# dremovd/PPO

Measured on AMD Instinct MI355X. Metric: env-steps/sec (Pong-shaped synthetic, 256 envs/GPU), higher is better.
Workload: dtype f32

## Files before the change

ppo_amd/csrc/stack_fused.hip:

```cpp
#include <cstdlib>
#include <type_traits>

#include "common.h"
#include "conv_stage.h"
#include "mfma.h"

#ifndef PPO_TAIL_SPLIT
#define PPO_TAIL_SPLIT 2
#endif

namespace ppo {
namespace {

constexpr int kScrPitchS = 20;

struct StackTailArgs {
    const float *in;
    const float *w[4];
    const float *bias[4];
    const float *mask[4];
    float *save[4];
    int n_images;
};

// ... 291 lines not shown

            __syncthreads();
#pragma unroll 1
            for (int hs = 0; hs <= S::NBANDS; ++hs) {
                if ((hs & 1) == grp) {
                    if (hs < S::NBANDS) {
                        const int y0 = hs * TR;
                        const int chan_off = ch * (H * W) + y0 * W;
#pragma unroll
                        for (int m = 0; m < MT; ++m) {
                            const bool live = p4[m] < S::NPIX;
                            const int off = live ? (chan_off + p4[m]) * 4 : kOutside;
                            if constexpr (BACKWARD) gate4[m] = buffer_f32x4(mask_b, off);
                            res4[m] = buffer_f32x4(res_b, off);
                        }
                        constexpr int CS_HI = ((C / 4 - 1) * 4 * PLANE + 2 * PITCH + 2) * 4 > 65535 ? C / 8 : C / 4;
                        static_assert(((C / 4 - 1 - (CS_HI < C / 4 ? CS_HI : 0)) * 4 * PLANE + 2 * PITCH + 2) * 4 <= 65535 &&
                                      ((CS_HI - 1) * 4 * PLANE + 2 * PITCH + 2) * 4 <= 65535, "operand offsets fit the instruction");
                        using lds_cvf = const volatile __attribute__((address_space(3))) float;
                        lds_cvf *vsmem = (lds_cvf *)smem;
                        int base[MT], base_hi[MT];
#pragma unroll
                        for (int m = 0; m < MT; ++m) {
                            base[m] = lofs[m] + (y0 - 1 + in_row) * PITCH;
                            base_hi[m] = base[m] + CS_HI * 4 * PLANE;
                            if constexpr (CS_HI < C / 4) asm volatile("" : "+v"(base_hi[m]));
                            acc[m] = f32x4{0.f, 0.f, 0.f, 0.f};
                        }
                        constexpr int SB = 2;
                        constexpr int NB = (KS + SB - 1) / SB;
                        float raw[2][SB][MT];
                        auto load_block = [&](int j, float (&r)[SB][MT]) {
#pragma unroll
                            for (int u = 0; u < SB; ++u) {
                                const int s = j * SB + u;
                                if (s < KS) {
                                    const int tap = s / (C / 4), cs = s % (C / 4);
                                    const int tap_off = (tap / 3) * PITCH + (tap % 3);
#pragma unroll
                                    for (int m = 0; m < MT; ++m)
                                        r[u][m] = cs < CS_HI ? vsmem[base[m] + cs * 4 * PLANE + tap_off]
                                                             : vsmem[base_hi[m] + (cs - CS_HI) * 4 * PLANE + tap_off];
                                }
                            }
                        };
                        load_block(0, raw[0]);
#pragma unroll
                        for (int j = 0; j < NB; ++j) {
                            __builtin_amdgcn_sched_barrier(0);
                            if (j + 1 < NB) load_block(j + 1, raw[(j + 1) & 1]);
                            __builtin_amdgcn_sched_barrier(0);
#pragma unroll
                            for (int u = 0; u < SB; ++u) {
                                const int s = j * SB + u;
                                if (s < KS) {
#pragma unroll
                                    for (int m = 0; m < MT; ++m) acc[m] = mfma16(wa[s], raw[j & 1][u][m], acc[m]);
                                }
                            }
                            __builtin_amdgcn_sched_barrier(0);
                        }
                    } else if (layer < 3) {
                        for (int i = tid % (S::GW * 64); i < C * W; i += S::GW * 64)
                            smem[(i / W) * PLANE + G + (H + in_row - 1) * PITCH + i % W] = 0.f;
                    }
                } else if (hs >= 1) {
                    const int y0 = (hs - 1) * TR;
                    const int chan_off = ch * (H * W) + y0 * W;
#pragma unroll
                    for (int m = 0; m < MT; ++m)
#pragma unroll
                        for (int r = 0; r < 4; ++r) scr[(m * 16 + g * 4 + r) * kScrPitchS + l15] = acc[m][r];
                    __builtin_amdgcn_wave_barrier();
                    float *out_row = smem + ch * PLANE + G + (y0 + in_row - 1) * PITCH;
#pragma unroll
                    for (int m = 0; m < MT; ++m) {
                        if (p4[m] >= S::NPIX) continue;
                        const float4 o = *reinterpret_cast<const float4 *>(scr + (m * 16 + ch) * kScrPitchS + quad * 4);
                        const float ov[4] = {o.x, o.y, o.z, o.w};
                        const float gv[4] = {gate4[m].x, gate4[m].y, gate4[m].z, gate4[m].w};
                        const float rv[4] = {res4[m].x, res4[m].y, res4[m].z, res4[m].w};
                        float v[4];
#pragma unroll
                        for (int e = 0; e < 4; ++e) {
                            float val = ov[e] + bias_c;
                            if constexpr (BACKWARD) val = gv[e] > 0.f ? val : 0.f;
                            v[e] = val + rv[e];
                        }
                        if (layer < 3) {
                            float t[4];
#pragma unroll
                            for (int e = 0; e < 4; ++e) t[e] = BACKWARD ? v[e] : relu1(v[e]);
                            *reinterpret_cast<float2 *>(out_row + po[m][0]) = make_float2(t[0], t[1]);
                            *reinterpret_cast<float2 *>(out_row + po[m][1]) = make_float2(t[2], t[3]);
                        }
                        if (save) *reinterpret_cast<float4 *>(save + chan_off + p4[m]) = make_float4(v[0], v[1], v[2], v[3]);
                    }
                    __builtin_amdgcn_wave_barrier();
                }
                __syncthreads();
            }
        }
    }
}

template <int C, int H, int W, int TR, bool BACKWARD>
int launch_stack_shift(const StackTailArgs &args, hipStream_t st)
{
    using S = ShiftCfg<C, H, W, TR>;
    constexpr auto kern = stack_shift_kernel<C, H, W, TR, BACKWARD>;
    if (int rc = prepare_kernel<kern>("stack_shift", S::LDS_BYTES)) return rc;
    int grid = 256;
    if (grid > args.n_images) grid = args.n_images;
    hipLaunchKernelGGL(kern, dim3(grid), dim3(S::NW * 64), S::LDS_BYTES, st, args);
    return check_launch("stack_shift_kernel");
}

template <int I, int N, class F>
__device__ __forceinline__ void static_for(F &&f)
{
    if constexpr (I < N) {
        f(std::integral_constant<int, I>{});
        static_for<I + 1, N>(f);
    }
}

struct LaneMap {
    template <int MT>
    struct T {
        int pix[MT], lofs[MT];
        float hi_l[MT], hi_r[MT];
    };
};

template <int H, int W, int PLANE, int G, int MT, int PITCH = W>
__device__ __forceinline__ void lane_map_init(LaneMap::T<MT> &lm, int pixel_wave, int l15, int g)
{
#pragma unroll
    for (int m = 0; m < MT; ++m) {
        const int p = (pixel_wave * MT + m) * 16 + l15;
        lm.pix[m] = p;
        const int pc = p < H * W ? p : 0;
        if constexpr (PITCH == W) {
            lm.lofs[m] = G + pc - 1 + g * PLANE;
            lm.hi_l[m] = (pc % W == 0) ? 0.f : INFINITY;
            lm.hi_r[m] = (pc % W == W - 1) ? 0.f : INFINITY;
        } else {
            lm.lofs[m] = G + (pc / W) * PITCH + pc % W - 1 + g * PLANE;
            lm.hi_l[m] = lm.hi_r[m] = 0.f;
        }
    }
}

template <int C, int H, int W, int MT, int NTOT, int NT, bool RELU_IN, bool GATED = false, int PITCH = W>
__device__ __forceinline__ void resident_conv(float *smem, int src_off, int dst_off, bool residual, const float *wpk,
                                              const float *bias, float *save, const LaneMap::T<MT> &lm, int n0, int lane,
                                              const float *mask = nullptr)
{
    constexpr int ROWS = H + 2, G = 4, PLANE_RAW = ROWS * PITCH + 2 * G;
    constexpr int PLANE = PLANE_RAW + ((16 - PLANE_RAW % 32) + 32) % 32;
    constexpr int KS = 9 * (C / 4);
    constexpr bool PADDED = PITCH != W;
    static_assert(!PADDED || (PITCH == W + 1 && !RELU_IN), "padded maps hold what the MFMA takes: identity input only");
    const int g = lane >> 4;
    float wa[NT][KS];
    const float4 *pw = reinterpret_cast<const float4 *>(wpk);
#pragma unroll
    for (int s4 = 0; s4 < KS / 4; ++s4)
#pragma unroll
        for (int n = 0; n < NT; ++n) {
            const float4 v = pw[(s4 * NTOT + n0 + n) * 64 + lane];
            wa[n][4 * s4 + 0] = v.x;
            wa[n][4 * s4 + 1] = v.y;
            wa[n][4 * s4 + 2] = v.z;
            wa[n][4 * s4 + 3] = v.w;
        }
    float bias_r[NT][4];
#pragma unroll
    for (int n = 0; n < NT; ++n)
#pragma unroll
        for (int r = 0; r < 4; ++r) bias_r[n][r] = (GATED || !bias) ? 0.f : bias[(n0 + n) * 16 + g * 4 + r];
    constexpr int SB = (MT * NT >= 4) ? 2 : 4;
    constexpr int NB = (KS + SB - 1) / SB;
    constexpr int GATE_AT = (GATED && MT * NT * 4 > 16) ? NB / 2 : -1;
    float gate[GATED ? MT : 1][NT][4];
    auto load_gate = [&]() {
        const __amdgpu_buffer_rsrc_t mask_b = buffer_of(mask);
#pragma unroll
        for (int m = 0; m < MT; ++m)
#pragma unroll
            for (int n = 0; n < NT; ++n)
#pragma unroll
                for (int r = 0; r < 4; ++r)
                    gate[m][n][r] = buffer_f32(mask_b, lm.pix[m] < H * W ? (((n0 + n) * 16 + g * 4 + r) * (H * W) + lm.pix[m]) * 4
                                                                         : kOutside);
    };
    if constexpr (GATED && GATE_AT < 0) load_gate();

    __syncthreads();
    int base[MT];
#pragma unroll
    for (int m = 0; m < MT; ++m) {
        base[m] = lm.lofs[m] + src_off;
        if constexpr (PADDED) asm volatile("" : "+v"(base[m]));
    }
    f32x4 acc[NT][MT];
#pragma unroll
    for (int n = 0; n < NT; ++n)
#pragma unroll
        for (int m = 0; m < MT; ++m) acc[n][m] = f32x4{0.f, 0.f, 0.f, 0.f};

    float raw[2][SB][MT];
    auto load_block = [&](int j, float (&r)[SB][MT]) {
#pragma unroll
        for (int u = 0; u < SB; ++u) {
            const int s = j * SB + u;
            if (s < KS) {
                const int tap = s / (C / 4), cs = s % (C / 4);
                const int tap_off = (tap / 3) * PITCH + (tap % 3);
#pragma unroll
                for (int m = 0; m < MT; ++m) {
                    if constexpr (PADDED) {
                        using lds_cvf = const volatile __attribute__((address_space(3))) float;
                        r[u][m] = ((lds_cvf *)smem)[base[m] + cs * 4 * PLANE + tap_off];
                    } else {
                        r[u][m] = smem[base[m] + cs * 4 * PLANE + tap_off];
                    }
                }
            }
        }
    };
    static_assert(!PADDED || ((C / 4 - 1) * 4 * PLANE + 2 * PITCH + 2) * 4 <= 65535, "operand offsets fit the instruction");
    load_block(0, raw[0]);
    static_for<0, NB>([&](auto jc) {
        constexpr int j = decltype(jc)::value;
        float bv[SB][MT];
#pragma unroll
        for (int u = 0; u < SB; ++u) {
            const int s = j * SB + u;
            if (s < KS) {
                const int kx = (s / (C / 4)) % 3;
#pragma unroll
                for (int m = 0; m < MT; ++m) {
                    float x = raw[j & 1][u][m];
                    if constexpr (PADDED) {
                    } else if (kx != 1) {
                        const float hi = kx == 0 ? lm.hi_l[m] : lm.hi_r[m];
                        x = __builtin_amdgcn_fmed3f(x, RELU_IN ? 0.f : -hi, hi);
                    } else if (RELU_IN) {
                        x = relu1(x);
                    }
                    bv[u][m] = x;
                }
            }
        }
        __builtin_amdgcn_sched_barrier(0);
        if constexpr (j + 1 < NB) load_block(j + 1, raw[(j + 1) & 1]);
        if constexpr (PADDED) __builtin_amdgcn_sched_barrier(0);
        if constexpr (j == GATE_AT) load_gate();
#pragma unroll
        for (int u = 0; u < SB; ++u) {
            const int s = j * SB + u;
            if (s < KS) {
#pragma unroll
                for (int m = 0; m < MT; ++m)
#pragma unroll
                    for (int n = 0; n < NT; ++n) acc[n][m] = mfma16(wa[n][s], bv[u][m], acc[n][m]);
            }
        }
        __builtin_amdgcn_sched_barrier(0);
    });
#pragma unroll
    for (int m = 0; m < MT; ++m) {
        if (lm.pix[m] < H * W) {
#pragma unroll
            for (int n = 0; n < NT; ++n)
#pragma unroll
                for (int r = 0; r < 4; ++r) {
                    const int co = (n0 + n) * 16 + g * 4 + r;
                    const int lo = PADDED ? dst_off + co * PLANE + (lm.lofs[m] - g * PLANE) + PITCH + 1
                                          : dst_off + co * PLANE + G + W + lm.pix[m];
                    float val = acc[n][m][r] + bias_r[n][r];
                    if constexpr (GATED) val = gate[m][n][r] > 0.f ? val : 0.f;
                    if (residual) val = val + smem[lo];
                    smem[lo] = val;
                    if (save) save[(size_t)co * (H * W) + lm.pix[m]] = val;
                }
        }
    }
}

struct StackFullArgs {
    const float *in;
    const float *w[5];
    const float *bias[5];
    float *pooled;
    uint8_t *argmax;
    float *save[4];
    const float *pre_w[4];
    const float *pre_bias[4];
    float *pre_save[4];
    int has_pre;
    int n_images;
};

template <int C, int HI, int WI, int MTI, int HO, int WO, int MTO, int NW, int NSPLIT>
__global__ __launch_bounds__(NW * NSPLIT * 64) void stack_full_kernel(StackFullArgs a)
{
    using SI = StackCfg<C, HI, WI, MTI, NW, NSPLIT>;
    using SO = StackCfg<C, HO, WO, MTO, NW, NSPLIT>;
    static_assert(HO == (HI + 1) / 2 && WO == (WI + 1) / 2, "3x3 / stride 2 / pad 1 pooling");
    static_assert(2 * SO::LDS_MAP <= SI::LDS_MAP, "the small maps reuse the input map's LDS");
    constexpr int NT = SI::NTL, WAVES = SI::WAVES, THREADS = WAVES * 64;
    constexpr int A_OFF = 0, B_OFF = SI::LDS_MAP, X_OFF = 0, Y_OFF = SO::LDS_MAP;
    extern __shared__ __align__(16) float smem[];
    const int tid = threadIdx.x, lane = tid & 63, l15 = lane & 15, g = lane >> 4;
    const int wave = tid >> 6, pixel_wave = wave % NW, n0 = (wave / NW) * NT;

    LaneMap::T<MTI> lmi;
    LaneMap::T<MTO> lmo;
    lane_map_init<HI, WI, SI::PLANE, SI::G, MTI>(lmi, pixel_wave, l15, g);
    lane_map_init<HO, WO, SO::PLANE, SO::G, MTO>(lmo, pixel_wave, l15, g);

    if (a.has_pre) zero_lds<SI::LDS_MAP, THREADS>(smem + B_OFF, tid);

    for (int img = blockIdx.x; img < a.n_images; img += gridDim.x) {
        __syncthreads();
        zero_lds<SI::LDS_MAP, THREADS>(smem + A_OFF, tid);
        __syncthreads();
        stage_band_chunk_dma<C, HI, WI, SI::ROWS, SI::PLANE, SI::G, WAVES>(a.in, img, 0, smem + A_OFF, tid);
        if (a.has_pre) {
            const size_t big_img = (size_t)img * C * HI * WI;
#pragma unroll 1
            for (int layer = 0; layer < 4; ++layer) {
                const int odd = layer & 1;
                float *save = a.pre_save[layer] ? a.pre_save[layer] + big_img : nullptr;
                resident_conv<C, HI, WI, MTI, SI::NT, NT, true>(smem, odd ? B_OFF : A_OFF, odd ? A_OFF : B_OFF, odd != 0,
                                                                a.pre_w[layer], a.pre_bias[layer], save, lmi, n0, lane);
            }
        }
        resident_conv<C, HI, WI, MTI, SI::NT, NT, false>(smem, A_OFF, B_OFF, false, a.w[0], a.bias[0], nullptr, lmi, n0, lane);
        __syncthreads();
        zero_lds<2 * SO::LDS_MAP, THREADS>(smem + X_OFF, tid);
        __syncthreads();
        {
            constexpr int RPW = 64 / WO;
            const int sub = lane / WO, xo = lane % WO;
            const size_t out_img = (size_t)img * C * HO * WO;
            for (int u0 = wave * RPW; u0 < C * HO; u0 += WAVES * RPW) {
                const int u = u0 + sub;
                const int co = u / HO, yo = u % HO;
                if (sub < RPW && co < C) {
                    const float *src = smem + B_OFF + co * SI::PLANE + SI::G + WI + (2 * yo - 1) * WI + 2 * xo - 1;
                    float best;
                    int best_tap;
                    pool_window_lds<HI % 2 == 0, WI % 2 == 0>(src, WI, yo > 0, 2 * yo + 1 < HI, xo > 0, 2 * xo + 1 < WI, best, best_tap);
                    smem[X_OFF + co * SO::PLANE + SO::G + WO + yo * WO + xo] = best;
                    const size_t oi = out_img + ((size_t)co * HO + yo) * WO + xo;
                    if (a.pooled) a.pooled[oi] = best;
                    if (a.argmax) a.argmax[oi] = (uint8_t)best_tap;
                }
            }
        }
        const size_t out_img = (size_t)img * C * HO * WO;
#pragma unroll 1
        for (int layer = 0; layer < 4; ++layer) {
            const int odd = layer & 1;
            float *save = a.save[layer] ? a.save[layer] + out_img : nullptr;
            resident_conv<C, HO, WO, MTO, SO::NT, NT, true>(smem, odd ? Y_OFF : X_OFF, odd ? X_OFF : Y_OFF, odd != 0,
                                                            a.w[1 + layer], a.bias[1 + layer], save, lmo, n0, lane);
        }
    }
}

struct StackFullBwdArgs {
    const float *g;
    const float *w[5];
    const float *mask[4];
    const uint8_t *argmax;
    float *save[4];
    float *dc;
    float *g_prev;
    const float *post_w[4];
    const float *post_mask[4];
    float *post_save[4];
    int has_post;
    int n_images;
};

template <int C, int HI, int WI, int MTI, int HO, int WO, int MTO, int NW, int NSPLIT>
__global__ __launch_bounds__(NW * NSPLIT * 64) void stack_full_bwd_kernel(StackFullBwdArgs a)
{
    using SI = StackCfg<C, HI, WI, MTI, NW, NSPLIT, WI + 1>;
    using SO = StackCfg<C, HO, WO, MTO, NW, NSPLIT, WO + 1>;
    static_assert(2 * SO::LDS_MAP <= SI::LDS_MAP, "the small maps live inside the first big map's LDS");
    static_assert(C * HO * WO <= SO::LDS_MAP * 4, "the argmax bytes of an image fit the second small map");
    constexpr int NT = SI::NTL, WAVES = SI::WAVES, THREADS = WAVES * 64;
    constexpr int A_OFF = 0, B_OFF = SI::LDS_MAP, X_OFF = 0, Y_OFF = SO::LDS_MAP;
    extern __shared__ __align__(16) float smem[];
    const int tid = threadIdx.x, lane = tid & 63, l15 = lane & 15, g = lane >> 4;
    const int wave = tid >> 6, pixel_wave = wave % NW, n0 = (wave / NW) * NT;

    LaneMap::T<MTI> lmi;
    LaneMap::T<MTO> lmo;
    lane_map_init<HI, WI, SI::PLANE, SI::G, MTI, SI::PITCH>(lmi, pixel_wave, l15, g);
    lane_map_init<HO, WO, SO::PLANE, SO::G, MTO, SO::PITCH>(lmo, pixel_wave, l15, g);

    zero_lds<SI::LDS_MAP, THREADS>(smem + B_OFF, tid);

    for (int img = blockIdx.x; img < a.n_images; img += gridDim.x) {
        __syncthreads();
        zero_lds<2 * SO::LDS_MAP, THREADS>(smem + X_OFF, tid);
        __syncthreads();
        const size_t small_img = (size_t)img * C * HO * WO, big_img = (size_t)img * C * HI * WI;
        for (int row = tid; row < C * HO; row += THREADS) {
            const float *gr = a.g + small_img + row * WO;
            float *lr = smem + X_OFF + (row / HO) * SO::PLANE + SO::G + (1 + row % HO) * SO::PITCH;
            float gv[WO];
#pragma unroll
            for (int x = 0; x < WO; ++x) gv[x] = gr[x];
#pragma unroll
            for (int x = 0; x < WO; ++x) lr[x] = gv[x];
        }
        constexpr int AM_WORDS = C * HO * WO / 4, AM_PER = (AM_WORDS + THREADS - 1) / THREADS;
        static_assert(C * HO * WO % 4 == 0, "an image's argmax bytes are whole words (the entry points check the base)");
        uint32_t am_r[AM_PER];
#pragma unroll
        for (int k = 0; k < AM_PER; ++k) {
            const int i = tid + k * THREADS;
            am_r[k] = reinterpret_cast<const uint32_t *>(a.argmax + small_img)[i < AM_WORDS ? i : 0];
        }
#pragma unroll 1
        for (int layer = 0; layer < 4; ++layer) {
            const int odd = layer & 1;
            resident_conv<C, HO, WO, MTO, SO::NT, NT, false, true, SO::PITCH>(smem, odd ? Y_OFF : X_OFF, odd ? X_OFF : Y_OFF, odd != 0,
                                                                   a.w[layer], nullptr, a.save[layer] + small_img, lmo, n0,
                                                                   lane, a.mask[layer] + small_img);
        }
        __syncthreads();
        const uint8_t *am = reinterpret_cast<const uint8_t *>(smem + Y_OFF);
#pragma unroll
        for (int k = 0; k < AM_PER; ++k) {
            const int i = tid + k * THREADS;
            if (i < AM_WORDS) reinterpret_cast<uint32_t *>(smem + Y_OFF)[i] = am_r[k];
        }
        __syncthreads();
        {
            for (int e = tid; e < C * HI * WI; e += THREADS) {
                const int co = e / (HI * WI), r = e % (HI * WI);
                const int iy = r / WI, ix = r % WI;
                const int k = ix >> 1, oy0 = iy >> 1;
                const int ky0 = (iy & 1) ? 2 : 1;
                const bool has_oy1 = (iy & 1) && (oy0 + 1 < HO);
                const bool odd_x = ix & 1;
                const bool has_ox1 = odd_x && (k + 1 < WO);
                const int kx0 = odd_x ? 2 : 1;
                const float *gx = smem + X_OFF + co * SO::PLANE + SO::G + SO::PITCH;
                const uint8_t *ac = am + co * (HO * WO);
                float sum = 0.f;
                {
                    const int i00 = oy0 * WO + k, x00 = oy0 * SO::PITCH + k;
                    if (ac[i00] == ky0 * 3 + kx0) sum += gx[x00];
                    if (has_ox1 && ac[i00 + 1] == ky0 * 3 + 0) sum += gx[x00 + 1];
                }
                if (has_oy1) {
                    const int i10 = (oy0 + 1) * WO + k, x10 = (oy0 + 1) * SO::PITCH + k;
                    if (ac[i10] == kx0) sum += gx[x10];
                    if (has_ox1 && ac[i10 + 1] == 0) sum += gx[x10 + 1];
                }
                smem[B_OFF + co * SI::PLANE + SI::G + (1 + iy) * SI::PITCH + ix] = sum;
                a.dc[big_img + e] = sum;
            }
        }
        if (a.has_post) {
            __syncthreads();
            zero_lds<SI::LDS_MAP, THREADS>(smem + A_OFF, tid);
        }
        resident_conv<C, HI, WI, MTI, SI::NT, NT, false, false, SI::PITCH>(smem, B_OFF, A_OFF, false, a.w[4], nullptr,
                                                                a.g_prev + big_img, lmi, n0, lane);
        if (a.has_post) {
#pragma unroll 1
            for (int layer = 0; layer < 4; ++layer) {
                const int odd = layer & 1;
                resident_conv<C, HI, WI, MTI, SI::NT, NT, false, true, SI::PITCH>(smem, odd ? B_OFF : A_OFF, odd ? A_OFF : B_OFF, odd != 0,
                                                                       a.post_w[layer], nullptr, a.post_save[layer] + big_img,
                                                                       lmi, n0, lane, a.post_mask[layer] + big_img);
            }
        }
    }
}

template <int C, int HI, int WI, int MTI, int HO, int WO, int MTO, int NW, int NSPLIT>
int launch_stack_full(const StackFullBwdArgs &args, hipStream_t st)
{
    using SI = StackCfg<C, HI, WI, MTI, NW, NSPLIT, WI + 1>;
    constexpr size_t kLds = 2 * (size_t)SI::LDS_MAP * 4;
    static_assert(kLds <= 160 * 1024, "two padded maps fit the CU's LDS");
    constexpr auto kern = stack_full_bwd_kernel<C, HI, WI, MTI, HO, WO, MTO, NW, NSPLIT>;
    if (int rc = prepare_kernel<kern>("stack_full_bwd", kLds)) return rc;
    const int grid = args.n_images < 256 ? args.n_images : 256;
    hipLaunchKernelGGL(kern, dim3(grid), dim3(SI::WAVES * 64), kLds, st, args);
    return check_launch("stack_full_bwd_kernel");
}

template <int C, int HI, int WI, int MTI, int HO, int WO, int MTO, int NW, int NSPLIT>
int launch_stack_full(const StackFullArgs &args, hipStream_t st)
{
    using SI = StackCfg<C, HI, WI, MTI, NW, NSPLIT>;
    constexpr size_t kLds = 2 * (size_t)SI::LDS_MAP * 4;
    constexpr auto kern = stack_full_kernel<C, HI, WI, MTI, HO, WO, MTO, NW, NSPLIT>;
    if (int rc = prepare_kernel<kern>("stack_full", kLds)) return rc;
    const int grid = args.n_images < 256 ? args.n_images : 256;
    hipLaunchKernelGGL(kern, dim3(grid), dim3(SI::WAVES * 64), kLds, st, args);
    return check_launch("stack_full_kernel");
}


struct ChainSplitArgs {
    const float *in;
    const float *pre_w[4];
    const float *pre_bias[4];
    const float *w[5];
    const float *bias[5];
    float *out;
    float *xbuf;
    uint32_t *flags;
    uint32_t *ctl;
    int n_images;
    int skip;
};

constexpr int kSplitWaves = 8;
constexpr uint32_t kSpinLimit = 1u << 21;

template <int C, int HI, int WI, int HO, int WO>
__global__ __launch_bounds__(kSplitWaves * 64) void stack_chain_split_kernel(ChainSplitArgs a)
{
    static_assert(C == 32, "two channel tiles: one per workgroup of a pair");
    using SI = StackCfg<C, HI, WI, 7, 4, 2>;
    using SO = StackCfg<C, HO, WO, 2, 4, 2>;
    constexpr int MTI = 4, MTO = 2, WAVES = kSplitWaves, THREADS = WAVES * 64;
    static_assert(SI::MTILES <= MTI * WAVES && SO::MTILES == MTO * 4 && WAVES == 8, "every pixel tile has a wave");
    static_assert(2 * SO::LDS_MAP <= SI::LDS_MAP, "the small maps reuse the input map's LDS");
    constexpr int A_OFF = 0, B_OFF = SI::LDS_MAP, X_OFF = 0, Y_OFF = SO::LDS_MAP;
    extern __shared__ __align__(16) float smem[];
    const int tid = threadIdx.x, lane = tid & 63, l15 = lane & 15, g = lane >> 4;
    const int wave = tid >> 6;
    const int b = blockIdx.x;
    const int h = (b >> 3) & 1;
    const int pair0 = (b & 7) | ((b >> 4) << 3);
    const int n_pairs = (gridDim.x >> 4) << 3;

    LaneMap::T<MTI> lmi;
    LaneMap::T<MTO> lmo;
    lane_map_init<HI, WI, SI::PLANE, SI::G, MTI>(lmi, wave, l15, g);
    lane_map_init<HO, WO, SO::PLANE, SO::G, MTO>(lmo, wave & 3, l15, g);

    const uint32_t base = __hip_atomic_load(a.ctl, __ATOMIC_RELAXED, __HIP_MEMORY_SCOPE_AGENT) * 8u;
    const uint32_t fault = __hip_atomic_load(a.ctl + 3, __ATOMIC_RELAXED, __HIP_MEMORY_SCOPE_AGENT);
    const uint32_t spin_limit = fault ? 1u << 10 : kSpinLimit;
    bool gave_up = false;
    zero_lds<SI::LDS_MAP, THREADS>(smem + B_OFF, tid);

    for (int img = pair0; img < a.n_images; img += n_pairs) {
        uint32_t *flag_own = a.flags + 2 * img + h, *flag_other = a.flags + 2 * img + (1 - h);
        float *slots = a.xbuf + (size_t)img * 2 * C * HI * WI;
        uint32_t step = 0;
        auto exchange = [&](int dst_off, float *slot, bool fetch) {
            ++step;
            asm volatile("s_waitcnt vmcnt(0)" ::: "memory");
            __syncthreads();
            if (tid == 0) {
                if (!(fault && h == 1))
                    __hip_atomic_store(flag_own, base + step, __ATOMIC_RELAXED, __HIP_MEMORY_SCOPE_AGENT);
                uint32_t it = 0;
                while (!(a.skip & 1) && !gave_up &&
                       __hip_atomic_load(flag_other, __ATOMIC_RELAXED, __HIP_MEMORY_SCOPE_AGENT) < base + step) {
                    if (++it > spin_limit ||
                        ((it & 1023u) == 0 && __hip_atomic_load(a.ctl + 2, __ATOMIC_RELAXED, __HIP_MEMORY_SCOPE_AGENT))) {
                        __hip_atomic_store(a.ctl + 2, 1u, __ATOMIC_RELAXED, __HIP_MEMORY_SCOPE_AGENT);
                        gave_up = true;
                        break;
                    }
                    __builtin_amdgcn_s_sleep(2);
                }
            }
            __syncthreads();
            if (fetch)
                stage_band_chunk_dma<16, HI, WI, SI::ROWS, SI::PLANE, SI::G, WAVES, 16>(slot + (size_t)(1 - h) * 16 * HI * WI, 0, 0,
                                                                                       smem + dst_off + (1 - h) * 16 * SI::PLANE, tid);
        };

        __syncthreads();
        zero_lds<SI::LDS_MAP, THREADS>(smem + A_OFF, tid);
        __syncthreads();
        stage_band_chunk_dma<C, HI, WI, SI::ROWS, SI::PLANE, SI::G, WAVES>(a.in, img, 0, smem + A_OFF, tid);
#pragma unroll 1
        for (int layer = 0; layer < 4; ++layer) {
            const int odd = layer & 1;
            float *slot = slots + (size_t)(layer & 1) * C * HI * WI;
            resident_conv<C, HI, WI, MTI, 2, 1, true>(smem, odd ? B_OFF : A_OFF, odd ? A_OFF : B_OFF, odd != 0, a.pre_w[layer],
                                                      a.pre_bias[layer], slot, lmi, h, lane);
            exchange(odd ? A_OFF : B_OFF, slot, true);
        }
        resident_conv<C, HI, WI, MTI, 2, 1, false>(smem, A_OFF, B_OFF, false, a.w[0], a.bias[0], slots, lmi, h, lane);
        exchange(B_OFF, slots, h == 0);
        if (h != 0 || (a.skip & 2)) continue;
        __syncthreads();
        zero_lds<2 * SO::LDS_MAP, THREADS>(smem + X_OFF, tid);
        __syncthreads();
        {
            constexpr int RPW = 64 / WO;
            const int sub = lane / WO, xo = lane % WO;
            for (int u0 = wave * RPW; u0 < C * HO; u0 += WAVES * RPW) {
                const int u = u0 + sub;
                const int co = u / HO, yo = u % HO;
                if (sub < RPW && co < C) {
                    const float *src = smem + B_OFF + co * SI::PLANE + SI::G + WI + (2 * yo - 1) * WI + 2 * xo - 1;
                    float best;
                    int best_tap;
                    pool_window_lds<HI % 2 == 0, WI % 2 == 0>(src, WI, yo > 0, 2 * yo + 1 < HI, xo > 0, 2 * xo + 1 < WI, best, best_tap);
                    smem[X_OFF + co * SO::PLANE + SO::G + WO + yo * WO + xo] = best;
                }
            }
        }
        float *out_img = a.out + (size_t)img * C * HO * WO;
#pragma unroll 1
        for (int layer = 0; layer < 4; ++layer) {
            const int odd = layer & 1;
            resident_conv<C, HO, WO, MTO, 2, 1, true>(smem, odd ? Y_OFF : X_OFF, odd ? X_OFF : Y_OFF, odd != 0, a.w[1 + layer],
                                                      a.bias[1 + layer], layer == 3 ? out_img : nullptr, lmo, wave >> 2, lane);
        }
    }
    __syncthreads();
    if (tid == 0) {
        const uint32_t done = __hip_atomic_fetch_add(a.ctl + 1, 1u, __ATOMIC_RELAXED, __HIP_MEMORY_SCOPE_AGENT);
        if (done == gridDim.x - 1) {
            __hip_atomic_store(a.ctl + 1, 0u, __ATOMIC_RELAXED, __HIP_MEMORY_SCOPE_AGENT);
            __hip_atomic_fetch_add(a.ctl, 1u, __ATOMIC_RELAXED, __HIP_MEMORY_SCOPE_AGENT);
        }
    }
}

template <int C, int HI, int WI, int HO, int WO>
int launch_chain_split(const ChainSplitArgs &args, hipStream_t st)
{
    using SI = StackCfg<C, HI, WI, 7, 4, 2>;
    constexpr size_t kLds = 2 * (size_t)SI::LDS_MAP * 4;
    constexpr auto kern = stack_chain_split_kernel<C, HI, WI, HO, WO>;
    if (int rc = prepare_kernel<kern>("stack_chain_split", kLds)) return rc;
    int groups = (args.n_images + 7) / 8;
    if (groups > 16) groups = 16;
    hipLaunchKernelGGL(kern, dim3(16 * groups), dim3(kSplitWaves * 64), kLds, st, args);
    return check_launch("stack_chain_split_kernel");
}

#define PPO_STACK_CASE(LAUNCH, C, H, W, ...) \
    if (channels == C && h == H && w == W) return args ? LAUNCH<C, H, W, __VA_ARGS__>(*args, st) : PPO_OK;

int no_kernel(const char *who, int channels, int h, int w)
{
    return fail(PPO_E_INVALID, "%s: no kernel for %d channels at %dx%d", who, channels, h, w);
}

template <bool BACKWARD>
int dispatch_stack_tail(const char *who, int channels, int h, int w, const StackTailArgs *args, hipStream_t st)
{
    PPO_STACK_CASE(launch_stack_shift, 16, 42, 42, 6, BACKWARD)
    PPO_STACK_CASE(launch_stack_shift, 16, 32, 32, 8, BACKWARD)
    PPO_STACK_CASE(launch_stack_tail, 32, 11, 11, 2, 4, PPO_TAIL_SPLIT, BACKWARD)
    PPO_STACK_CASE(launch_stack_tail, 32, 21, 21, 7, 4, PPO_TAIL_SPLIT, BACKWARD)
    PPO_STACK_CASE(launch_stack_tail, 32, 16, 16, 4, 4, PPO_TAIL_SPLIT, BACKWARD)
    PPO_STACK_CASE(launch_stack_tail, 32, 8, 8, 1, 4, PPO_TAIL_SPLIT, BACKWARD)
    return args ? no_kernel(who, channels, h, w) : PPO_E_INVALID;
}

template <class Args>
int dispatch_stack_full(const char *who, int channels, int h, int w, const Args *args, hipStream_t st)
{
    PPO_STACK_CASE(launch_stack_full, 32, 21, 21, 7, 11, 11, 2, 4, 2)
    PPO_STACK_CASE(launch_stack_full, 32, 16, 16, 4, 8, 8, 1, 4, 2)
    return args ? no_kernel(who, channels, h, w) : PPO_E_INVALID;
}

int dispatch_chain_split(const char *who, int channels, int h, int w, const ChainSplitArgs *args, hipStream_t st)
{
    PPO_STACK_CASE(launch_chain_split, 32, 21, 21, 11, 11)
    return args ? no_kernel(who, channels, h, w) : PPO_E_INVALID;
}
#undef PPO_STACK_CASE

template <int N, int M>
int fill_layers(const char *who, const char *other, const float *const *weights, const float *const *others,
                const float *(&w)[N], const float *(&o)[M])
{
    for (int l = 0; l < N; ++l) {
        if (!weights[l] || (l < M && !others[l])) return fail(PPO_E_INVALID, "%s: null weights / %s of layer %d", who, other, l);
        if (!aligned(weights[l], 16)) return fail(PPO_E_ALIGN, "%s: packed weights must be 16-byte aligned", who);
        w[l] = weights[l];
        if (l < M) o[l] = others[l];
    }
    return PPO_OK;
}

struct ChainedStack {
    const float *const *weights, *const *others;
    float *save[4];
};

int stack_full_forward(const char *who, const float *in, const ChainedStack *pre, const float *const *packed_weights,
                       const float *const *biases, float *pooled, uint8_t *argmax, float *a0, float *q0, float *a1, float *q1,
                       int n_images, int channels, int h, int w, void *stream)
{
    if (n_images < 0) return fail(PPO_E_INVALID, "%s: negative batch", who);
    if (n_images == 0) return PPO_OK;
    if (!in || !packed_weights || !biases || !q1 || (pre && (!pre->weights || !pre->others)))
        return fail(PPO_E_INVALID, "%s: null pointer", who);
    StackFullArgs args{};
    args.in = in, args.pooled = pooled, args.argmax = argmax, args.n_images = n_images;
    args.save[0] = a0, args.save[1] = q0, args.save[2] = a1, args.save[3] = q1;
    if (int rc = fill_layers(who, "bias", packed_weights, biases, args.w, args.bias)) return rc;
    if (pre) {
        if (int rc = fill_layers(who, "bias", pre->weights, pre->others, args.pre_w, args.pre_bias)) return rc;
        for (int l = 0; l < 4; ++l) args.pre_save[l] = pre->save[l];
        args.has_pre = 1;
    }
    return dispatch_stack_full(who, channels, h, w, &args, as_stream(stream));
}

int stack_full_backward(const char *who, const float *g, const float *const *packed_weights_t, const float *const *masks,
                        const uint8_t *argmax, float *da1, float *g1, float *da0, float *g0, float *dc, float *g_prev,
                        const ChainedStack *post, int n_images, int channels, int h, int w, void *stream)
{
    if (n_images < 0) return fail(PPO_E_INVALID, "%s: negative batch", who);
    if (n_images == 0) return PPO_OK;
    if (!g || !packed_weights_t || !masks || !argmax || !da1 || !g1 || !da0 || !g0 || !dc || !g_prev ||
        (post && (!post->weights || !post->others || !post->save[0] || !post->save[1] || !post->save[2] || !post->save[3])))
        return fail(PPO_E_INVALID, "%s: null pointer", who);
    if (!aligned(argmax, 4)) return fail(PPO_E_ALIGN, "%s: argmax must be 4-byte aligned", who);
    StackFullBwdArgs args{};
    args.g = g, args.argmax = argmax, args.dc = dc, args.g_prev = g_prev, args.n_images = n_images;
    args.save[0] = da1, args.save[1] = g1, args.save[2] = da0, args.save[3] = g0;
    if (int rc = fill_layers(who, "mask", packed_weights_t, masks, args.w, args.mask)) return rc;
    if (post) {
        if (int rc = fill_layers(who, "mask", post->weights, post->others, args.post_w, args.post_mask)) return rc;
        for (int l = 0; l < 4; ++l) args.post_save[l] = post->save[l];
        args.has_post = 1;
    }
    return dispatch_stack_full(who, channels, h, w, &args, as_stream(stream));
}

struct ChainSplitLayout {
    size_t flags, ctl, bytes;
};
ChainSplitLayout chain_split_layout(int n_images, int channels, int h, int w)
{
    const size_t slots = (size_t)n_images * 2 * channels * h * w * sizeof(float);
    const size_t flags = ((size_t)n_images * 2 * sizeof(uint32_t) + 15) & ~(size_t)15;
    return {slots, slots + flags, slots + flags + 16};
}

}
}

extern "C" int ppo_impala_stack_tail_supported(int channels, int h, int w)
{
    return ppo::dispatch_stack_tail<false>(nullptr, channels, h, w, nullptr, nullptr) == PPO_OK;
}

extern "C" int ppo_impala_stack_tail_forward_f32(const float *in, const float *const *packed_weights,
                                                 const float *const *biases, float *a0, float *q0, float *a1, float *q1,
                                                 int n_images, int channels, int h, int w, void *stream)
{
    using namespace ppo;
    const char *who = "ppo_impala_stack_tail_forward_f32";
    if (n_images < 0) return fail(PPO_E_INVALID, "%s: negative batch", who);
    if (n_images == 0) return PPO_OK;
    if (!in || !packed_weights || !biases || !q1) return fail(PPO_E_INVALID, "%s: null pointer", who);
    StackTailArgs args{};
    args.in = in, args.n_images = n_images;
    args.save[0] = a0, args.save[1] = q0, args.save[2] = a1, args.save[3] = q1;
    if (int rc = fill_layers(who, "bias", packed_weights, biases, args.w, args.bias)) return rc;
    if (!aligned(in, 4)) return fail(PPO_E_ALIGN, "%s: input must be 4-byte aligned", who);
    if (channels == 16) {
// ... 108 lines not shown
```

Before: 98480.

## Prefetch next layer's weights during conv epilogue and switch forward maps to padded layout

Weight and bias loading is split out of resident_conv into a ConvOperand held in registers. Each conv now prefetches the next layer's (or next image's) weights before its epilogue, so global weight latency overlaps the store phase. The forward stack kernel also moves to padded-pitch LDS maps with ReLU applied on output, which drops the per-tap edge clamping, and it stages input through registers instead of the DMA helper. This costs more register pressure and makes the layer-chaining logic more intricate.

```diff
diff --git a/ppo_amd/csrc/stack_fused.hip b/ppo_amd/csrc/stack_fused.hip
--- a/ppo_amd/csrc/stack_fused.hip
+++ b/ppo_amd/csrc/stack_fused.hip
@@ -467,34 +467,55 @@
     }
 }
 
-template <int C, int H, int W, int MT, int NTOT, int NT, bool RELU_IN, bool GATED = false, int PITCH = W>
-__device__ __forceinline__ void resident_conv(float *smem, int src_off, int dst_off, bool residual, const float *wpk,
-                                              const float *bias, float *save, const LaneMap::T<MT> &lm, int n0, int lane,
-                                              const float *mask = nullptr)
+template <int C, int NT>
+struct ConvOperand {
+    float wa[NT][9 * (C / 4)];
+    float bias[NT][4];
+};
+
+template <int C, int NTOT, int NT, bool BIAS>
+__device__ __forceinline__ void load_conv_operand(ConvOperand<C, NT> &op, const float *wpk, const float *bias, int n0, int lane)
+{
+    const int g = lane >> 4;
+#pragma unroll
+    for (int n = 0; n < NT; ++n)
+#pragma unroll
+        for (int r = 0; r < 4; ++r) {
+            if constexpr (BIAS) op.bias[n][r] = bias[(n0 + n) * 16 + g * 4 + r];
+            else op.bias[n][r] = 0.f;
+        }
+    const float4 *pw = reinterpret_cast<const float4 *>(wpk);
+#pragma unroll
+    for (int s4 = 0; s4 < 9 * (C / 4) / 4; ++s4)
+#pragma unroll
+        for (int n = 0; n < NT; ++n) {
+            const float4 v = pw[(s4 * NTOT + n0 + n) * 64 + lane];
+            op.wa[n][4 * s4 + 0] = v.x;
+            op.wa[n][4 * s4 + 1] = v.y;
+            op.wa[n][4 * s4 + 2] = v.z;
+            op.wa[n][4 * s4 + 3] = v.w;
+        }
+}
+
+template <int C, int H, int W, int MT, int NTOT, int NT, bool RELU_IN, bool GATED = false, int PITCH = W, bool BIAS = !GATED,
+          bool RELU_OUT = false>
+__device__ __forceinline__ void resident_conv(float *smem, int src_off, int dst_off, bool residual, ConvOperand<C, NT> &op,
+                                              const float *next_w, const float *next_bias, int next_n0, float *save,
+                                              const LaneMap::T<MT> &lm, int n0, int lane, const float *mask = nullptr)
 {
     constexpr int ROWS = H + 2, G = 4, PLANE_RAW = ROWS * PITCH + 2 * G;
     constexpr int PLANE = PLANE_RAW + ((16 - PLANE_RAW % 32) + 32) % 32;
     constexpr int KS = 9 * (C / 4);
     constexpr bool PADDED = PITCH != W;
-    static_assert(!PADDED || (PITCH == W + 1 && !RELU_IN), "padded maps hold what the MFMA takes: identity input only");
+    static_assert(!PADDED || PITCH == W + 1, "one zero float behind every row");
+    static_assert(!RELU_OUT || (PADDED && !GATED), "pre-activated results belong to the padded forward maps");
     const int g = lane >> 4;
-    float wa[NT][KS];
-    const float4 *pw = reinterpret_cast<const float4 *>(wpk);
-#pragma unroll
-    for (int s4 = 0; s4 < KS / 4; ++s4)
-#pragma unroll
-        for (int n = 0; n < NT; ++n) {
-            const float4 v = pw[(s4 * NTOT + n0 + n) * 64 + lane];
-            wa[n][4 * s4 + 0] = v.x;
-            wa[n][4 * s4 + 1] = v.y;
-            wa[n][4 * s4 + 2] = v.z;
-            wa[n][4 * s4 + 3] = v.w;
-        }
+    float (&wa)[NT][KS] = op.wa;
     float bias_r[NT][4];
 #pragma unroll
     for (int n = 0; n < NT; ++n)
 #pragma unroll
-        for (int r = 0; r < 4; ++r) bias_r[n][r] = (GATED || !bias) ? 0.f : bias[(n0 + n) * 16 + g * 4 + r];
+        for (int r = 0; r < 4; ++r) bias_r[n][r] = op.bias[n][r];
     constexpr int SB = (MT * NT >= 4) ? 2 : 4;
     constexpr int NB = (KS + SB - 1) / SB;
     constexpr int GATE_AT = (GATED && MT * NT * 4 > 16) ? NB / 2 : -1;
@@ -559,6 +580,7 @@
                 for (int m = 0; m < MT; ++m) {
                     float x = raw[j & 1][u][m];
                     if constexpr (PADDED) {
+                        if constexpr (RELU_IN) asm("v_med3_f32 %0, %1, 0, %2" : "=v"(x) : "v"(x), "s"(0x7f800000));
                     } else if (kx != 1) {
                         const float hi = kx == 0 ? lm.hi_l[m] : lm.hi_r[m];
                         x = __builtin_amdgcn_fmed3f(x, RELU_IN ? 0.f : -hi, hi);
@@ -585,6 +607,8 @@
         }
         __builtin_amdgcn_sched_barrier(0);
     });
+    if (next_w) load_conv_operand<C, NTOT, NT, BIAS>(op, next_w, next_bias, next_n0, lane);
+    __builtin_amdgcn_sched_barrier(0);
 #pragma unroll
     for (int m = 0; m < MT; ++m) {
         if (lm.pix[m] < H * W) {
@@ -598,7 +622,7 @@
                     float val = acc[n][m][r] + bias_r[n][r];
                     if constexpr (GATED) val = gate[m][n][r] > 0.f ? val : 0.f;
                     if (residual) val = val + smem[lo];
-                    smem[lo] = val;
+                    smem[lo] = RELU_OUT ? relu1(val) : val;
                     if (save) save[(size_t)co * (H * W) + lm.pix[m]] = val;
                 }
         }
@@ -622,8 +646,8 @@
 template <int C, int HI, int WI, int MTI, int HO, int WO, int MTO, int NW, int NSPLIT>
 __global__ __launch_bounds__(NW * NSPLIT * 64) void stack_full_kernel(StackFullArgs a)
 {
-    using SI = StackCfg<C, HI, WI, MTI, NW, NSPLIT>;
-    using SO = StackCfg<C, HO, WO, MTO, NW, NSPLIT>;
+    using SI = StackCfg<C, HI, WI, MTI, NW, NSPLIT, WI + 1>;
+    using SO = StackCfg<C, HO, WO, MTO, NW, NSPLIT, WO + 1>;
     static_assert(HO == (HI + 1) / 2 && WO == (WI + 1) / 2, "3x3 / stride 2 / pad 1 pooling");
     static_assert(2 * SO::LDS_MAP <= SI::LDS_MAP, "the small maps reuse the input map's LDS");
     constexpr int NT = SI::NTL, WAVES = SI::WAVES, THREADS = WAVES * 64;
@@ -634,27 +658,49 @@
 
     LaneMap::T<MTI> lmi;
     LaneMap::T<MTO> lmo;
-    lane_map_init<HI, WI, SI::PLANE, SI::G, MTI>(lmi, pixel_wave, l15, g);
-    lane_map_init<HO, WO, SO::PLANE, SO::G, MTO>(lmo, pixel_wave, l15, g);
+    lane_map_init<HI, WI, SI::PLANE, SI::G, MTI, SI::PITCH>(lmi, pixel_wave, l15, g);
+    lane_map_init<HO, WO, SO::PLANE, SO::G, MTO, SO::PITCH>(lmo, pixel_wave, l15, g);
 
     if (a.has_pre) zero_lds<SI::LDS_MAP, THREADS>(smem + B_OFF, tid);
 
+    ConvOperand<C, NT> op;
+    const float *first_w = a.has_pre ? a.pre_w[0] : a.w[0], *first_bias = a.has_pre ? a.pre_bias[0] : a.bias[0];
+    if ((int)blockIdx.x < a.n_images) load_conv_operand<C, SI::NT, NT, true>(op, first_w, first_bias, n0, lane);
+
     for (int img = blockIdx.x; img < a.n_images; img += gridDim.x) {
+        const size_t big_img = (size_t)img * C * HI * WI;
+        constexpr int IN_WORDS = C * HI * WI, IN_PER = (IN_WORDS + THREADS - 1) / THREADS;
+        float in_r[IN_PER];
+#pragma unroll
+        for (int k = 0; k < IN_PER; ++k) {
+            const int i = tid + k * THREADS;
+            in_r[k] = a.in[big_img + (i < IN_WORDS ? i : 0)];
+        }
         __syncthreads();
         zero_lds<SI::LDS_MAP, THREADS>(smem + A_OFF, tid);
         __syncthreads();
-        stage_band_chunk_dma<C, HI, WI, SI::ROWS, SI::PLANE, SI::G, WAVES>(a.in, img, 0, smem + A_OFF, tid);
-        if (a.has_pre) {
-            const size_t big_img = (size_t)img * C * HI * WI;
+        int tid_s = tid;
+        asm volatile("" : "+v"(tid_s));
+#pragma unroll
+        for (int k = 0; k < IN_PER; ++k) {
+            const int i = tid_s + k * THREADS;
+            const int c = i / (HI * WI), r = i % (HI * WI);
+            if (i < IN_WORDS) smem[A_OFF + c * SI::PLANE + SI::G + SI::PITCH + r + r / WI] = in_r[k];
+        }
 #pragma unroll 1
-            for (int layer = 0; layer < 4; ++layer) {
-                const int odd = layer & 1;
-                float *save = a.pre_save[layer] ? a.pre_save[layer] + big_img : nullptr;
-                resident_conv<C, HI, WI, MTI, SI::NT, NT, true>(smem, odd ? B_OFF : A_OFF, odd ? A_OFF : B_OFF, odd != 0,
-                                                                a.pre_w[layer], a.pre_bias[layer], save, lmi, n0, lane);
-            }
-        }
-        resident_conv<C, HI, WI, MTI, SI::NT, NT, false>(smem, A_OFF, B_OFF, false, a.w[0], a.bias[0], nullptr, lmi, n0, lane);
+        for (int i = a.has_pre ? 0 : 2; i < 3; ++i) {
+            if (i < 2) {
+                float *save = a.pre_save[2 * i] ? a.pre_save[2 * i] + big_img : nullptr;
+                resident_conv<C, HI, WI, MTI, SI::NT, NT, true, false, SI::PITCH, true, true>(
+                    smem, A_OFF, B_OFF, false, op, a.pre_w[2 * i + 1], a.pre_bias[2 * i + 1], n0, save, lmi, n0, lane);
+            }
+            const bool first = i == 2;
+            float *save1 = first ? nullptr : a.pre_save[2 * i + 1];
+            if (save1) save1 += big_img;
+            resident_conv<C, HI, WI, MTI, SI::NT, NT, false, false, SI::PITCH>(
+                smem, first ? A_OFF : B_OFF, first ? B_OFF : A_OFF, !first, op, first ? a.w[1] : i == 0 ? a.pre_w[2] : a.w[0],
+                first ? a.bias[1] : i == 0 ? a.pre_bias[2] : a.bias[0], n0, save1, lmi, n0, lane);
+        }
         __syncthreads();
         zero_lds<2 * SO::LDS_MAP, THREADS>(smem + X_OFF, tid);
         __syncthreads();
@@ -666,11 +712,12 @@
                 const int u = u0 + sub;
                 const int co = u / HO, yo = u % HO;
                 if (sub < RPW && co < C) {
-                    const float *src = smem + B_OFF + co * SI::PLANE + SI::G + WI + (2 * yo - 1) * WI + 2 * xo - 1;
+                    const float *src = smem + B_OFF + co * SI::PLANE + SI::G + 2 * yo * SI::PITCH + 2 * xo - 1;
                     float best;
                     int best_tap;
-                    pool_window_lds<HI % 2 == 0, WI % 2 == 0>(src, WI, yo > 0, 2 * yo + 1 < HI, xo > 0, 2 * xo + 1 < WI, best, best_tap);
-                    smem[X_OFF + co * SO::PLANE + SO::G + WO + yo * WO + xo] = best;
+                    pool_window_lds<HI % 2 == 0, WI % 2 == 0>(src, SI::PITCH, yo > 0, 2 * yo + 1 < HI, xo > 0, 2 * xo + 1 < WI, best,
+                                                              best_tap);
+                    smem[X_OFF + co * SO::PLANE + SO::G + (1 + yo) * SO::PITCH + xo] = best;
                     const size_t oi = out_img + ((size_t)co * HO + yo) * WO + xo;
                     if (a.pooled) a.pooled[oi] = best;
                     if (a.argmax) a.argmax[oi] = (uint8_t)best_tap;
@@ -678,12 +725,16 @@
             }
         }
         const size_t out_img = (size_t)img * C * HO * WO;
+        const float *next_img_w = img + (int)gridDim.x < a.n_images ? first_w : nullptr;
 #pragma unroll 1
-        for (int layer = 0; layer < 4; ++layer) {
-            const int odd = layer & 1;
-            float *save = a.save[layer] ? a.save[layer] + out_img : nullptr;
-            resident_conv<C, HO, WO, MTO, SO::NT, NT, true>(smem, odd ? Y_OFF : X_OFF, odd ? X_OFF : Y_OFF, odd != 0,
-                                                            a.w[1 + layer], a.bias[1 + layer], save, lmo, n0, lane);
+        for (int blk = 0; blk < 2; ++blk) {
+            float *save0 = a.save[2 * blk] ? a.save[2 * blk] + out_img : nullptr;
+            float *save1 = a.save[2 * blk + 1] ? a.save[2 * blk + 1] + out_img : nullptr;
+            resident_conv<C, HO, WO, MTO, SO::NT, NT, true, false, SO::PITCH, true, true>(
+                smem, X_OFF, Y_OFF, false, op, a.w[2 + 2 * blk], a.bias[2 + 2 * blk], n0, save0, lmo, n0, lane);
+            resident_conv<C, HO, WO, MTO, SO::NT, NT, false, false, SO::PITCH>(
+                smem, Y_OFF, X_OFF, true, op, blk == 0 ? a.w[3] : next_img_w, blk == 0 ? a.bias[3] : first_bias, n0, save1, lmo, n0,
+                lane);
         }
     }
 }
@@ -723,7 +774,11 @@
 
     zero_lds<SI::LDS_MAP, THREADS>(smem + B_OFF, tid);
 
+    ConvOperand<C, NT> op;
+    if ((int)blockIdx.x < a.n_images) load_conv_operand<C, SI::NT, NT, false>(op, a.w[0], nullptr, n0, lane);
+
     for (int img = blockIdx.x; img < a.n_images; img += gridDim.x) {
+        const float *next_img_w = img + (int)gridDim.x < a.n_images ? a.w[0] : nullptr;
         __syncthreads();
         zero_lds<2 * SO::LDS_MAP, THREADS>(smem + X_OFF, tid);
         __syncthreads();
@@ -749,8 +804,8 @@
         for (int layer = 0; layer < 4; ++layer) {
             const int odd = layer & 1;
             resident_conv<C, HO, WO, MTO, SO::NT, NT, false, true, SO::PITCH>(smem, odd ? Y_OFF : X_OFF, odd ? X_OFF : Y_OFF, odd != 0,
-                                                                   a.w[layer], nullptr, a.save[layer] + small_img, lmo, n0,
-                                                                   lane, a.mask[layer] + small_img);
+                                                                   op, a.w[layer + 1], nullptr, n0, a.save[layer] + small_img,
+                                                                   lmo, n0, lane, a.mask[layer] + small_img);
         }
         __syncthreads();
         const uint8_t *am = reinterpret_cast<const uint8_t *>(smem + Y_OFF);
@@ -791,15 +846,17 @@
             __syncthreads();
             zero_lds<SI::LDS_MAP, THREADS>(smem + A_OFF, tid);
         }
-        resident_conv<C, HI, WI, MTI, SI::NT, NT, false, false, SI::PITCH>(smem, B_OFF, A_OFF, false, a.w[4], nullptr,
+        resident_conv<C, HI, WI, MTI, SI::NT, NT, false, false, SI::PITCH, false>(smem, B_OFF, A_OFF, false, op,
+                                                                a.has_post ? a.post_w[0] : next_img_w, nullptr, n0,
                                                                 a.g_prev + big_img, lmi, n0, lane);
         if (a.has_post) {
 #pragma unroll 1
             for (int layer = 0; layer < 4; ++layer) {
                 const int odd = layer & 1;
                 resident_conv<C, HI, WI, MTI, SI::NT, NT, false, true, SI::PITCH>(smem, odd ? B_OFF : A_OFF, odd ? A_OFF : B_OFF, odd != 0,
-                                                                       a.post_w[layer], nullptr, a.post_save[layer] + big_img,
-                                                                       lmi, n0, lane, a.post_mask[layer] + big_img);
+                                                                       op, layer < 3 ? a.post_w[layer + 1] : next_img_w, nullptr, n0,
+                                                                       a.post_save[layer] + big_img, lmi, n0, lane,
+                                                                       a.post_mask[layer] + big_img);
             }
         }
     }
@@ -821,8 +878,9 @@
 template <int C, int HI, int WI, int MTI, int HO, int WO, int MTO, int NW, int NSPLIT>
 int launch_stack_full(const StackFullArgs &args, hipStream_t st)
 {
-    using SI = StackCfg<C, HI, WI, MTI, NW, NSPLIT>;
+    using SI = StackCfg<C, HI, WI, MTI, NW, NSPLIT, WI + 1>;
     constexpr size_t kLds = 2 * (size_t)SI::LDS_MAP * 4;
+    static_assert(kLds <= 160 * 1024, "two padded maps fit the CU's LDS");
     constexpr auto kern = stack_full_kernel<C, HI, WI, MTI, HO, WO, MTO, NW, NSPLIT>;
     if (int rc = prepare_kernel<kern>("stack_full", kLds)) return rc;
     const int grid = args.n_images < 256 ? args.n_images : 256;
@@ -876,6 +934,8 @@
     const uint32_t spin_limit = fault ? 1u << 10 : kSpinLimit;
     bool gave_up = false;
     zero_lds<SI::LDS_MAP, THREADS>(smem + B_OFF, tid);
+
+    ConvOperand<C, 1> op;
 
     for (int img = pair0; img < a.n_images; img += n_pairs) {
         uint32_t *flag_own = a.flags + 2 * img + h, *flag_other = a.flags + 2 * img + (1 - h);
@@ -914,11 +974,13 @@
         for (int layer = 0; layer < 4; ++layer) {
             const int odd = layer & 1;
             float *slot = slots + (size_t)(layer & 1) * C * HI * WI;
-            resident_conv<C, HI, WI, MTI, 2, 1, true>(smem, odd ? B_OFF : A_OFF, odd ? A_OFF : B_OFF, odd != 0, a.pre_w[layer],
-                                                      a.pre_bias[layer], slot, lmi, h, lane);
+            load_conv_operand<C, 2, 1, true>(op, a.pre_w[layer], a.pre_bias[layer], h, lane);
+            resident_conv<C, HI, WI, MTI, 2, 1, true>(smem, odd ? B_OFF : A_OFF, odd ? A_OFF : B_OFF, odd != 0, op, nullptr, nullptr,
+                                                      0, slot, lmi, h, lane);
             exchange(odd ? A_OFF : B_OFF, slot, true);
         }
-        resident_conv<C, HI, WI, MTI, 2, 1, false>(smem, A_OFF, B_OFF, false, a.w[0], a.bias[0], slots, lmi, h, lane);
+        load_conv_operand<C, 2, 1, true>(op, a.w[0], a.bias[0], h, lane);
+        resident_conv<C, HI, WI, MTI, 2, 1, false>(smem, A_OFF, B_OFF, false, op, nullptr, nullptr, 0, slots, lmi, h, lane);
         exchange(B_OFF, slots, h == 0);
         if (h != 0 || (a.skip & 2)) continue;
         __syncthreads();
@@ -943,8 +1005,9 @@
 #pragma unroll 1
         for (int layer = 0; layer < 4; ++layer) {
             const int odd = layer & 1;
-            resident_conv<C, HO, WO, MTO, 2, 1, true>(smem, odd ? Y_OFF : X_OFF, odd ? X_OFF : Y_OFF, odd != 0, a.w[1 + layer],
-                                                      a.bias[1 + layer], layer == 3 ? out_img : nullptr, lmo, wave >> 2, lane);
+            load_conv_operand<C, 2, 1, true>(op, a.w[1 + layer], a.bias[1 + layer], wave >> 2, lane);
+            resident_conv<C, HO, WO, MTO, 2, 1, true>(smem, odd ? Y_OFF : X_OFF, odd ? X_OFF : Y_OFF, odd != 0, op, nullptr, nullptr,
+                                                      0, layer == 3 ? out_img : nullptr, lmo, wave >> 2, lane);
         }
     }
     __syncthreads();
```

Measured after the change: 97330. -1.2%, worse.
